# george-gca/sr-pytorch-lightning

Measured on AMD Instinct MI355X. Metric: SR training throughput, LR patches/s (48x48 LR x4, fwd+bwd+Adam), higher is better.
Workload: dtype bf16; 1 GPU; edsr_baseline x4, 48x48 LR patches, batch 256/GPU, train step (L1 + Adam); global_batch=256, parallelism=dp1, hip_graph=full

## Files before the change

sr-pytorch-lightning_amd/csrc/hr_tail.hip:

```cpp
#include "srk_common.h"

namespace {

SRK_DEV void sub_of(int a, int d, int& i, int& s) {
  const int ap = a + d;
  i = ap & 1;
  s = (ap - i) >> 1;
}

struct Wts {
  const float* wt; const float* bt; const float* wu; const float* bu;
  int O, C, Ci;
};

SRK_DEV float sum16(float v) {
  v += __shfl_xor(v, 8, 64);
  v += __shfl_xor(v, 4, 64);
  v += __shfl_xor(v, 2, 64);
  v += __shfl_xor(v, 1, 64);
  return v;
}

SRK_DEV float collapse_w(const Wts& p, int sub, int o, int a, int b, int ci, int dy0, int dy1, int dx0, int dx1, int fy, int fx) {
  float acc = 0.f;
  for (int dy = dy0; dy <= dy1; ++dy) {
    int i, sy; sub_of(a, dy, i, sy);
    const int ey = fy - sy;
    if (ey < -1 || ey > 1) continue;
    for (int dx = dx0; dx <= dx1; ++dx) {
      int j, sx; sub_of(b, dx, j, sx);
      const int ex = fx - sx;
      if (ex < -1 || ex > 1) continue;
      const float* wt = p.wt + (size_t)o * p.C * 9 + (dy + 1) * 3 + (dx + 1);
      const float* wu = p.wu + ((size_t)(i * 2 + j) * p.Ci + ci) * 9 + (ey + 1) * 3 + (ex + 1);
      for (int c0 = sub; c0 < p.C; c0 += 64) {
        float x[4], y[4];
#pragma unroll
        for (int k = 0; k < 4; ++k) {
          const int c = c0 + 16 * k;
          const bool ok = c < p.C;
          x[k] = ok ? wt[(size_t)c * 9] : 0.f;
          y[k] = ok ? wu[(size_t)c * 4 * p.Ci * 9] : 0.f;
        }
#pragma unroll
        for (int k = 0; k < 4; ++k)
          if (c0 + 16 * k < p.C) acc += x[k] * y[k];
      }
    }
  }
  return sum16(acc);
}
SRK_DEV float collapse_b(const Wts& p, int sub, int o, int a, int b, int dy0, int dy1, int dx0, int dx1) {
  float acc = 0.f;
  if (p.bu) {
    for (int dy = dy0; dy <= dy1; ++dy) {
      int i, sy; sub_of(a, dy, i, sy);
      for (int dx = dx0; dx <= dx1; ++dx) {
        int j, sx; sub_of(b, dx, j, sx);
        const float* wt = p.wt + (size_t)o * p.C * 9 + (dy + 1) * 3 + (dx + 1);
        for (int c = sub; c < p.C; c += 16) acc += wt[(size_t)c * 9] * p.bu[c * 4 + i * 2 + j];
      }
    }
  }
  return sum16(acc);
}

__global__ __launch_bounds__(256) void hrtail_collapse_kernel(const srk_hrtail_args a) {
  const Wts p{a.wt, a.bt, a.wu, a.bu, a.O, a.C, a.Ci};
  const int O = a.O, Ci = a.Ci;
  const int n_eff = 4 * O * Ci * 25, n_edge = 4 * 2 * O * Ci * 5, n_cor = 4 * O * Ci;
  const int n_b = 4 * O + 4 * 2 * O + 4 * O;
  const int sub = threadIdx.x & 15;
  int t = blockIdx.x * 16 + (threadIdx.x >> 4);
  if (t >= n_eff + n_edge + n_cor + n_b) t = n_eff + n_edge + n_cor + n_b;
  float v = 0.f;
  float* dst = nullptr;
  if (t < n_eff) {
    const int f = t % 25, ci = (t / 25) % Ci, k = t / (25 * Ci);
    v = collapse_w(p, sub, k >> 2, (k >> 1) & 1, k & 1, ci, -1, 1, -1, 1, f / 5 - 2, f % 5 - 2);
    dst = a.weff + t;
  } else if (t < n_eff + n_edge) {
    const int u = t - n_eff;
    const int tt = u % 5, ci = (u / 5) % Ci, kk = (u / (5 * Ci)) % (2 * O), ty = u / (5 * Ci * 2 * O);
    const int o = kk >> 1, q = kk & 1;
    if (ty == 0) v = collapse_w(p, sub, o, 0, q, ci, -1, -1, -1, 1, 0, tt - 2);
    else if (ty == 1) v = collapse_w(p, sub, o, 1, q, ci, 1, 1, -1, 1, 0, tt - 2);
    else if (ty == 2) v = collapse_w(p, sub, o, q, 0, ci, -1, 1, -1, -1, tt - 2, 0);
    else v = collapse_w(p, sub, o, q, 1, ci, -1, 1, 1, 1, tt - 2, 0);
    dst = a.wedge + u;
  } else if (t < n_eff + n_edge + n_cor) {
    const int u = t - n_eff - n_edge;
    const int ci = u % Ci, o = (u / Ci) % O, c = u / (Ci * O);
    const int ca = c >> 1, cb = c & 1;
    v = collapse_w(p, sub, o, ca, cb, ci, ca ? 1 : -1, ca ? 1 : -1, cb ? 1 : -1, cb ? 1 : -1, 0, 0);
    dst = a.wcor + u;
  } else if (t < n_eff + n_edge + n_cor + n_b) {
    const int w = t - n_eff - n_edge - n_cor;
    if (w < 4 * O) {
      const int k = w;
      v = (a.bt ? a.bt[k >> 2] : 0.f) + collapse_b(p, sub, k >> 2, (k >> 1) & 1, k & 1, -1, 1, -1, 1);
      dst = a.beff + k;
    } else if (w < 4 * O + 8 * O) {
      const int u = w - 4 * O, kk = u % (2 * O), ty = u / (2 * O), o = kk >> 1, q = kk & 1;
      if (ty == 0) v = collapse_b(p, sub, o, 0, q, -1, -1, -1, 1);
      else if (ty == 1) v = collapse_b(p, sub, o, 1, q, 1, 1, -1, 1);
      else if (ty == 2) v = collapse_b(p, sub, o, q, 0, -1, 1, -1, -1);
      else v = collapse_b(p, sub, o, q, 1, -1, 1, 1, 1);
      dst = a.bedge + u;
    } else {
      const int u = w - 12 * O, o = u % O, c = u / O, ca = c >> 1, cb = c & 1;
      v = collapse_b(p, sub, o, ca, cb, ca ? 1 : -1, ca ? 1 : -1, cb ? 1 : -1, cb ? 1 : -1);
      dst = a.bcor + u;
    }
  }
  if (dst && sub == 0) *dst = v;
}

template <int DT> SRK_DEV float ld_act(const void* base, size_t idx) {
  return DTraits<DT>::to_f32(reinterpret_cast<const typename DTraits<DT>::elem*>(base)[idx]);
}

constexpr int MAXO = 4;
SRK_DEV float wave_total(float v) {
#pragma unroll
  for (int m = 32; m >= 1; m >>= 1) v += __shfl_xor(v, m, 64);
  return v;
}
struct EdgeGeo {
  int ty, len; bool row;
  int fix_lr, fix_hr;
};
SRK_DEV EdgeGeo edge_geo(int ty, int H, int W) {
  EdgeGeo e;
  e.ty = ty; e.row = ty < 2; e.len = e.row ? W : H;
  e.fix_lr = ty == 0 ? 0 : ty == 1 ? H - 1 : ty == 2 ? 0 : W - 1;
  e.fix_hr = ty == 0 ? 0 : ty == 1 ? 2 * H - 1 : ty == 2 ? 0 : 2 * W - 1;
  return e;
}
SRK_DEV void stage_copy256(float* __restrict__ dst, const float* __restrict__ src, int n) {
  int i = threadIdx.x;
  for (; i + 256 * 7 < n; i += 256 * 8) {
    float v[8];
#pragma unroll
    for (int k = 0; k < 8; ++k) v[k] = src[i + 256 * k];
#pragma unroll
    for (int k = 0; k < 8; ++k) dst[i + 256 * k] = v[k];
  }
  float v[8];
#pragma unroll
  for (int k = 0; k < 8; ++k) v[k] = i + 256 * k < n ? src[i + 256 * k] : 0.f;
#pragma unroll
  for (int k = 0; k < 8; ++k)
    if (i + 256 * k < n) dst[i + 256 * k] = v[k];
}
template <int DT>
SRK_DEV void stage_line(const srk_hrtail_args& a, const EdgeGeo& e, int n, float* Xl, int pitch) {
  typedef DTraits<DT> Tr;
  const int Ci = a.Ci;
  if ((Ci & 7) == 0 && (a.x_pitch & 7) == 0) {
    const int nch = Ci >> 3, total = (e.len + 4) * nch;
    for (int i0 = threadIdx.x; i0 < total; i0 += 256 * 4) {
      i32x4 raw[4];
#pragma unroll
      for (int u = 0; u < 4; ++u) {
        const int i = i0 + 256 * u;
        const int sp = i / nch, c8 = i - sp * nch, s = sp - 2;
        raw[u] = i32x4{0, 0, 0, 0};
        if (i < total && s >= 0 && s < e.len) {
          const int yy = e.row ? e.fix_lr : s, xx = e.row ? s : e.fix_lr;
          raw[u] = gload16(reinterpret_cast<const typename Tr::elem*>(a.x) + ((size_t)(n * a.H + yy) * a.W + xx) * a.x_pitch + c8 * 8);
        }
      }
#pragma unroll
      for (int u = 0; u < 4; ++u) {
        const int i = i0 + 256 * u;
        if (i >= total) continue;
        const int sp = i / nch, c8 = i - sp * nch;
        const int w4[4] = {raw[u].x, raw[u].y, raw[u].z, raw[u].w};
        float v[8];
#pragma unroll
        for (int k = 0; k < 4; ++k) unpack2<DT>((uint32_t)w4[k], v[2 * k], v[2 * k + 1]);
#pragma unroll
        for (int k = 0; k < 8; ++k) Xl[sp * pitch + c8 * 8 + k] = v[k];
      }
    }
    return;
  }
  for (int i = threadIdx.x; i < (e.len + 4) * Ci; i += 256) {
    const int s = i / Ci - 2, ci = i % Ci;
    float v = 0.f;
    if (s >= 0 && s < e.len) {
      const int yy = e.row ? e.fix_lr : s, xx = e.row ? s : e.fix_lr;
      v = ld_act<DT>(a.x, ((size_t)(n * a.H + yy) * a.W + xx) * a.x_pitch + ci);
    }
    Xl[(s + 2) * pitch + ci] = v;
  }
}

template <int DT>
__global__ __launch_bounds__(256) void hrtail_edge_fwd_kernel(const srk_hrtail_args a, int phase) {
  const int H = a.H, W = a.W, O = a.O, Ci = a.Ci, H2 = 2 * H, W2 = 2 * W;
  const int n = blockIdx.x;
  const EdgeGeo e = edge_geo(2 * phase + blockIdx.y, H, W);
  extern __shared__ __attribute__((aligned(16))) char smem_raw[];
  const int pitch = Ci + 1;
  float* const Xl = reinterpret_cast<float*>(smem_raw);
  float* const Wl = Xl + (size_t)(e.len + 4) * pitch;
  stage_line<DT>(a, e, n, Xl, pitch);
  stage_copy256(Wl, a.wedge + (size_t)e.ty * 2 * O * Ci * 5, 2 * O * Ci * 5);
  __syncthreads();
  const size_t oplane = (size_t)H2 * W2;
  float* const out = a.out + (size_t)n * O * oplane;
  for (int idx = threadIdx.x + 256 * blockIdx.z; idx < 2 * e.len * O; idx += 256 * gridDim.z) {
    const int p = idx % (2 * e.len), o = idx / (2 * e.len);
    const int s = p >> 1, q = p & 1;
    const float* const w = Wl + (size_t)(o * 2 + q) * Ci * 5;
    const float* const x = Xl + (size_t)s * pitch;
    float a0 = a.bedge[e.ty * 2 * O + o * 2 + q], a1 = 0.f, a2 = 0.f, a3 = 0.f, a4 = 0.f;
    for (int ci = 0; ci < Ci; ++ci) {
      a0 += w[ci * 5 + 0] * x[0 * pitch + ci]; a1 += w[ci * 5 + 1] * x[1 * pitch + ci]; a2 += w[ci * 5 + 2] * x[2 * pitch + ci];
      a3 += w[ci * 5 + 3] * x[3 * pitch + ci]; a4 += w[ci * 5 + 4] * x[4 * pitch + ci];
    }
    float acc = ((a0 + a1) + (a2 + a3)) + a4;
    if (!e.row && (p == 0 || p == 2 * e.len - 1)) {
      const int ca = p == 0 ? 0 : 1, cb = e.ty == 2 ? 0 : 1, c = ca * 2 + cb;
      float cc = a.bcor[c * O + o];
      const float* const xc = Xl + (size_t)(s + 2) * pitch;
      for (int ci = 0; ci < Ci; ++ci) cc += a.wcor[((size_t)c * O + o) * Ci + ci] * xc[ci];
      acc -= cc;
    }
    const size_t at = e.row ? (size_t)e.fix_hr * W2 + p : (size_t)p * W2 + e.fix_hr;
    out[(size_t)o * oplane + at] -= acc;
  }
}

template <int DT>
__global__ __launch_bounds__(256) void hrtail_edge_bwd_x_kernel(const srk_hrtail_args a, int phase) {
  typedef DTraits<DT> Tr;
  const int H = a.H, W = a.W, O = a.O, Ci = a.Ci, H2 = 2 * H, W2 = 2 * W;
  const int n = blockIdx.x;
  const bool shared_line = phase == 0 ? H == 1 : W == 1;
  if (shared_line && blockIdx.y == 1) return;
  extern __shared__ __attribute__((aligned(16))) char smem_raw[];
  const size_t gplane = (size_t)H2 * W2;
  const float* const g = a.g + (size_t)n * O * gplane;
  for (int rep = 0; rep < (shared_line ? 2 : 1); ++rep) {
  const EdgeGeo e = edge_geo(2 * phase + (shared_line ? rep : (int)blockIdx.y), H, W);
  float* const Gl = reinterpret_cast<float*>(smem_raw);
  float* const Wl = Gl + (size_t)2 * O * (e.len + 4);
  __syncthreads();
  for (int i0 = threadIdx.x; i0 < 2 * O * (e.len + 4); i0 += 256 * 4) {
    float v[4];
#pragma unroll
    for (int u = 0; u < 4; ++u) {
      const int i = i0 + 256 * u;
      const int kk = i / (e.len + 4), s = i % (e.len + 4) - 2, o = kk >> 1, q = kk & 1;
      v[u] = 0.f;
      if (i < 2 * O * (e.len + 4) && s >= 0 && s < e.len)
        v[u] = e.row ? g[(size_t)o * gplane + (size_t)e.fix_hr * W2 + 2 * s + q] : g[(size_t)o * gplane + (size_t)(2 * s + q) * W2 + e.fix_hr];
    }
#pragma unroll
    for (int u = 0; u < 4; ++u)
      if (i0 + 256 * u < 2 * O * (e.len + 4)) Gl[i0 + 256 * u] = v[u];
  }
  stage_copy256(Wl, a.wedge + (size_t)e.ty * 2 * O * Ci * 5, 2 * O * Ci * 5);
  __syncthreads();
  const int nch = (Ci + 7) >> 3;
  const bool vec = (Ci & 7) == 0 && (a.dx_pitch & 7) == 0;
  for (int idx = threadIdx.x + 256 * blockIdx.z; idx < e.len * nch; idx += 256 * gridDim.z) {
    const int c8 = idx % nch, s = idx / nch;
    float corr[8];
#pragma unroll
    for (int k = 0; k < 8; ++k) corr[k] = 0.f;
    for (int kk = 0; kk < 2 * O; ++kk) {
      const float* const gl = Gl + (size_t)kk * (e.len + 4) + s + 2;
      float gv[5];
#pragma unroll
      for (int tt = 0; tt < 5; ++tt) gv[tt] = gl[2 - tt];
#pragma unroll
      for (int k = 0; k < 8; ++k) {
        const int ci = c8 * 8 + k;
        if (ci < Ci) {
          const float* const w = Wl + ((size_t)kk * Ci + ci) * 5;
#pragma unroll
          for (int tt = 0; tt < 5; ++tt) corr[k] += w[tt] * gv[tt];
        }
      }
    }
    if (!e.row && (s == 0 || s == e.len - 1)) {
      for (int ca = 0; ca < 2; ++ca) {
        if (!(ca ? s == e.len - 1 : s == 0)) continue;
        const int cb = e.ty == 2 ? 0 : 1, c = ca * 2 + cb;
        const size_t at = (size_t)(ca ? H2 - 1 : 0) * W2 + e.fix_hr;
        for (int o = 0; o < O; ++o) {
          const float gc = g[(size_t)o * gplane + at];
#pragma unroll
          for (int k = 0; k < 8; ++k)
            if (c8 * 8 + k < Ci) corr[k] -= a.wcor[((size_t)c * O + o) * Ci + c8 * 8 + k] * gc;
        }
      }
    }
    const int yy = e.row ? e.fix_lr : s, xx = e.row ? s : e.fix_lr;
    typename Tr::elem* const d = reinterpret_cast<typename Tr::elem*>(a.dx) + ((size_t)(n * H + yy) * W + xx) * a.dx_pitch + c8 * 8;
    if (vec) {
      const i32x4 raw = *reinterpret_cast<const i32x4*>(d);
      const int w4[4] = {raw.x, raw.y, raw.z, raw.w};
      int o4[4];
#pragma unroll
      for (int k = 0; k < 4; ++k) {
        float f0, f1;
        unpack2<DT>((uint32_t)w4[k], f0, f1);
        o4[k] = (int)pack2<DT>(f0 - corr[2 * k], f1 - corr[2 * k + 1]);
      }
      *reinterpret_cast<i32x4*>(d) = i32x4{o4[0], o4[1], o4[2], o4[3]};
    } else {
#pragma unroll
      for (int k = 0; k < 8; ++k)
        if (c8 * 8 + k < Ci) d[k] = Tr::from_f32(Tr::to_f32(d[k]) - corr[k]);
    }
  }
  }
}

constexpr int EW_MAXLEN = 512;
template <int DT>
__global__ __launch_bounds__(256) void hrtail_edge_bwd_w_kernel(const srk_hrtail_args a, int nchunks, int ew_chunk) {
  const int H = a.H, W = a.W, O = a.O, Ci = a.Ci, H2 = 2 * H, W2 = 2 * W;
  const int ty = blockIdx.y, chunk = blockIdx.x;
  const int n0 = chunk * ew_chunk, n1 = min(a.N, n0 + ew_chunk);
  const int ncombo = ty < 4 ? 2 * O * 5 : O;
  const size_t gplane = (size_t)H2 * W2;
  float* const dst = a.scratch + ((size_t)ty * nchunks + chunk) * (size_t)(2 * MAXO * 5) * (Ci + 1);
  extern __shared__ __attribute__((aligned(16))) char smem_raw[];
  float* const Xl = reinterpret_cast<float*>(smem_raw);
  if (ty >= 4) {
    if (blockIdx.z != 0) return;
    const int c = ty - 4, ca = c >> 1, cbb = c & 1;
    const int Py = ca ? H2 - 1 : 0, Px = cbb ? W2 - 1 : 0, yy = ca ? H - 1 : 0, xx = cbb ? W - 1 : 0;
    for (int item = threadIdx.x; item < ncombo * (Ci + 1); item += 256) {
      const int ci = item % (Ci + 1), o = item / (Ci + 1);
      float acc = 0.f;
      for (int n = n0; n < n1; ++n) {
        const float gv = a.g[((size_t)n * O + o) * gplane + (size_t)Py * W2 + Px];
        const float xv = ci < Ci ? ld_act<DT>(a.x, ((size_t)(n * H + yy) * W + xx) * a.x_pitch + ci) : 1.f;
        acc += gv * xv;
      }
      dst[item] = acc;
    }
    return;
  }
  const bool rowedge = ty < 2;
  const int len = rowedge ? W : H;
  float* const Gl = Xl + (size_t)(len + 4) * Ci;
  constexpr int MAXIT = (2 * MAXO * 5 * 65 + 255) / 256;
  const int nitems = ncombo * (Ci + 1);
  const int ipb = (nitems + gridDim.z - 1) / gridDim.z, item0 = blockIdx.z * ipb, item1 = min(nitems, item0 + ipb);
  float acc[MAXIT];
#pragma unroll
  for (int k = 0; k < MAXIT; ++k) acc[k] = 0.f;
  for (int n = n0; n < n1; ++n) {
    __syncthreads();
    stage_line<DT>(a, edge_geo(ty, H, W), n, Xl, Ci);
    for (int i = threadIdx.x; i < 2 * O * len; i += 256) {
      const int kk = i / len, s = i % len, o = kk >> 1, q = kk & 1;
      const float* const g = a.g + ((size_t)n * O + o) * gplane;
      Gl[i] = rowedge ? g[(size_t)(ty == 0 ? 0 : H2 - 1) * W2 + 2 * s + q] : g[(size_t)(2 * s + q) * W2 + (ty == 2 ? 0 : W2 - 1)];
    }
    __syncthreads();
#pragma unroll
    for (int k = 0; k < MAXIT; ++k) {
      const int item = item0 + threadIdx.x + k * 256;
      if (item >= item1) break;
      const int ci = item % (Ci + 1), cb = item / (Ci + 1), tt = cb % 5, kk = cb / 5;
      const float* const gr = Gl + kk * len;
      float t0 = 0.f, t1 = 0.f, t2 = 0.f, t3 = 0.f;
      int p = 0;
      if (ci < Ci) {
        const float* const xr = Xl + (size_t)tt * Ci + ci;
        for (; p + 3 < len; p += 4) {
          t0 += gr[p] * xr[(size_t)p * Ci]; t1 += gr[p + 1] * xr[(size_t)(p + 1) * Ci];
          t2 += gr[p + 2] * xr[(size_t)(p + 2) * Ci]; t3 += gr[p + 3] * xr[(size_t)(p + 3) * Ci];
        }
        for (; p < len; ++p) t0 += gr[p] * xr[(size_t)p * Ci];
      } else if (tt == 2) {
        for (; p + 3 < len; p += 4) { t0 += gr[p]; t1 += gr[p + 1]; t2 += gr[p + 2]; t3 += gr[p + 3]; }
        for (; p < len; ++p) t0 += gr[p];
      }
      acc[k] += (t0 + t1) + (t2 + t3);
    }
  }
#pragma unroll
  for (int k = 0; k < MAXIT; ++k) {
    const int item = item0 + threadIdx.x + k * 256;
    if (item < item1) dst[item] = acc[k];
  }
}

__global__ __launch_bounds__(256) void hrtail_edge_reduce_kernel(const srk_hrtail_args a, int nchunks) {
  const int O = a.O, Ci = a.Ci;
  const int per = 2 * MAXO * 5 * (Ci + 1);
  const int t = blockIdx.x * 256 + threadIdx.x;
  const int n_edge = 4 * 2 * O * 5 * (Ci + 1), n_cor = 4 * O * (Ci + 1);
  if (t >= n_edge + n_cor) return;
  int ty, item;
  if (t < n_edge) { ty = t / (2 * O * 5 * (Ci + 1)); item = t % (2 * O * 5 * (Ci + 1)); }
  else { const int u = t - n_edge; ty = 4 + u / (O * (Ci + 1)); item = u % (O * (Ci + 1)); }
  const float* const src = a.scratch + (size_t)ty * nchunks * per + item;
  float s0 = 0.f, s1 = 0.f, s2 = 0.f, s3 = 0.f;
  int c = 0;
  for (; c + 3 < nchunks; c += 4) {
    s0 += src[(size_t)c * per]; s1 += src[(size_t)(c + 1) * per]; s2 += src[(size_t)(c + 2) * per]; s3 += src[(size_t)(c + 3) * per];
  }
  for (; c < nchunks; ++c) s0 += src[(size_t)c * per];
  const float s = (s0 + s1) + (s2 + s3);
  const int ci = item % (Ci + 1), cb = item / (Ci + 1);
  if (ty < 4) {
    const int tt = cb % 5, kk = cb / 5;
    if (ci < Ci) a.eedge[(((size_t)ty * 2 * O + kk) * Ci + ci) * 5 + tt] = s;
    else if (tt == 2) a.e0[ty * 2 * O + kk] = s;
  } else {
    if (ci < Ci) a.ecor[((size_t)(ty - 4) * O + cb) * Ci + ci] = s;
    else a.k0[(ty - 4) * O + cb] = s;
  }
}

struct Gr {
  const float* r; const float* r0; const float* ee; const float* e0; const float* ec; const float* k0;
  int O, Ci;
};
SRK_DEV int row_type(int a, int dy) { return (a == 0 && dy == -1) ? 0 : ((a == 1 && dy == 1) ? 1 : -1); }
SRK_DEV int col_type(int b, int dx) { return (b == 0 && dx == -1) ? 2 : ((b == 1 && dx == 1) ? 3 : -1); }
SRK_DEV float g_w(const Gr& q, int o, int a, int b, int dy, int dx, int ci, int fy, int fx) {
  float v = q.r[(((size_t)(o * 4 + a * 2 + b)) * q.Ci + ci) * 25 + (fy + 2) * 5 + (fx + 2)];
  const int rt = row_type(a, dy), ct = col_type(b, dx);
  if (rt >= 0 && fy == 0) v -= q.ee[(((size_t)rt * 2 * q.O + o * 2 + b) * q.Ci + ci) * 5 + fx + 2];
  if (ct >= 0 && fx == 0) v -= q.ee[(((size_t)ct * 2 * q.O + o * 2 + a) * q.Ci + ci) * 5 + fy + 2];
  if (rt >= 0 && ct >= 0 && fy == 0 && fx == 0) v += q.ec[((size_t)(a * 2 + b) * q.O + o) * q.Ci + ci];
  return v;
}
SRK_DEV float g_b(const Gr& q, int o, int a, int b, int dy, int dx) {
  float v = q.r0[o * 4 + a * 2 + b];
  const int rt = row_type(a, dy), ct = col_type(b, dx);
  if (rt >= 0) v -= q.e0[rt * 2 * q.O + o * 2 + b];
  if (ct >= 0) v -= q.e0[ct * 2 * q.O + o * 2 + a];
  if (rt >= 0 && ct >= 0) v += q.k0[(a * 2 + b) * q.O + o];
  return v;
}

__global__ __launch_bounds__(256) void hrtail_expand_kernel(const srk_hrtail_args a) {
  const Gr q{a.r, a.r0, a.eedge, a.e0, a.ecor, a.k0, a.O, a.Ci};
  const int O = a.O, C = a.C, Ci = a.Ci;
  const int n_wu = 4 * C * Ci * 9, n_bu = 4 * C, n_bt = O;
  const int nb_thread = (n_wu + n_bu + n_bt + 255) / 256;
  if ((int)blockIdx.x >= nb_thread) {
    const int t = ((int)blockIdx.x - nb_thread) * 4 + (threadIdx.x >> 6), lane = threadIdx.x & 63;
    if (t >= O * C * 9) return;
    const int d = t % 9, c = (t / 9) % C, o = t / (9 * C);
    const int dy = d / 3 - 1, dx = d % 3 - 1;
    float acc = 0.f;
    for (int pa = 0; pa < 2; ++pa) {
      int i, sy; sub_of(pa, dy, i, sy);
      for (int pb = 0; pb < 2; ++pb) {
        int j, sx; sub_of(pb, dx, j, sx);
        const int cu = c * 4 + i * 2 + j;
        if (a.bu && lane == 0) acc += g_b(q, o, pa, pb, dy, dx) * a.bu[cu];
        for (int ci = lane; ci < Ci; ci += 64)
#pragma unroll
          for (int e = 0; e < 9; ++e)
            acc += g_w(q, o, pa, pb, dy, dx, ci, sy + e / 3 - 1, sx + e % 3 - 1) * a.wu[((size_t)cu * Ci + ci) * 9 + e];
      }
    }
    acc = wave_total(acc);
    if (lane == 0) a.dwt[t] = acc;
    return;
  }
  int t = blockIdx.x * 256 + threadIdx.x;
  if (t < n_wu) {
    const int e = t % 9, ci = (t / 9) % Ci, cu = t / (9 * Ci), c = cu >> 2, i = (cu >> 1) & 1, j = cu & 1;
    const int ey = e / 3 - 1, ex = e % 3 - 1;
    float acc = 0.f;
    for (int pa = 0; pa < 2; ++pa)
      for (int dy = -1; dy <= 1; ++dy) {
        int ii, sy; sub_of(pa, dy, ii, sy);
        if (ii != i) continue;
        for (int pb = 0; pb < 2; ++pb)
          for (int dx = -1; dx <= 1; ++dx) {
            int jj, sx; sub_of(pb, dx, jj, sx);
            if (jj != j) continue;
            for (int o = 0; o < O; ++o)
              acc += a.wt[((size_t)o * C + c) * 9 + (dy + 1) * 3 + dx + 1] * g_w(q, o, pa, pb, dy, dx, ci, sy + ey, sx + ex);
          }
      }
    a.dwu[t] = acc;
    return;
  }
  t -= n_wu;
  if (t < n_bu) {
    if (!a.dbu) return;
    const int cu = t, c = cu >> 2, i = (cu >> 1) & 1, j = cu & 1;
    float acc = 0.f;
    for (int pa = 0; pa < 2; ++pa)
      for (int dy = -1; dy <= 1; ++dy) {
        int ii, sy; sub_of(pa, dy, ii, sy);
        if (ii != i) continue;
        for (int pb = 0; pb < 2; ++pb)
          for (int dx = -1; dx <= 1; ++dx) {
            int jj, sx; sub_of(pb, dx, jj, sx);
            if (jj != j) continue;
            for (int o = 0; o < O; ++o) acc += a.wt[((size_t)o * C + c) * 9 + (dy + 1) * 3 + dx + 1] * g_b(q, o, pa, pb, dy, dx);
          }
      }
    a.dbu[cu] = acc;
    return;
  }
  t -= n_bu;
  if (t < n_bt && a.dbt) a.dbt[t] = a.r0[t * 4] + a.r0[t * 4 + 1] + a.r0[t * 4 + 2] + a.r0[t * 4 + 3];
}

int check_common(const srk_hrtail_args* a, const char* who) {
  SRK_CHECK_ARG(a, "%s: null argument", who);
  SRK_CHECK_ARG(a->O >= 1 && a->O <= MAXO && a->C >= 1 && a->Ci >= 1, "%s: O=%d (1..%d) C=%d Ci=%d", who, a->O, MAXO, a->C, a->Ci);
  return 0;
}
int check_act(const srk_hrtail_args* a, const char* who) {
  SRK_CHECK_ARG(a->N > 0 && a->H > 0 && a->W > 0, "%s: bad dims N=%d H=%d W=%d", who, a->N, a->H, a->W);
  SRK_CHECK_ARG(a->dtype == SRK_BF16 || a->dtype == SRK_F16, "%s: 16-bit activations only", who);
  SRK_CHECK_ARG((long long)a->N * a->O * 4 * a->H * a->W < (1ll << 31), "%s: output too large", who);
  return 0;
}

}

extern "C" int srk_hrtail_collapse(const srk_hrtail_args* a, srk_stream_t stream) {
  if (int rc = check_common(a, "srk_hrtail_collapse")) return rc;
  SRK_CHECK_ARG(a->wt && a->wu && a->weff && a->beff && a->wedge && a->bedge && a->wcor && a->bcor, "srk_hrtail_collapse: null pointer");
  const int total = 4 * a->O * a->Ci * 25 + 4 * 2 * a->O * a->Ci * 5 + 4 * a->O * a->Ci + 16 * a->O;
  hipLaunchKernelGGL(hrtail_collapse_kernel, dim3((unsigned)((total + 15) / 16)), dim3(256), 0, reinterpret_cast<hipStream_t>(stream), *a);
  SRK_LAUNCH_CHECK();
  return 0;
}

static unsigned edge_split(int N) {
  const int z = (512 + 2 * N - 1) / (2 * N);
  return (unsigned)(z < 1 ? 1 : (z > 8 ? 8 : z));
}

template <typename K> static int edge_lds_attr(K kernel, const char* who) {
  const hipError_t e = hipFuncSetAttribute(reinterpret_cast<const void*>(kernel), hipFuncAttributeMaxDynamicSharedMemorySize, 160 * 1024);
  if (e != hipSuccess) { srk_set_error("%s: cannot reserve LDS: %s", who, hipGetErrorString(e)); return (int)e; }
  return 0;
}

extern "C" int srk_hrtail_edge_fwd(const srk_hrtail_args* a, srk_stream_t stream) {
  if (int rc = check_common(a, "srk_hrtail_edge_fwd")) return rc;
  if (int rc = check_act(a, "srk_hrtail_edge_fwd")) return rc;
  SRK_CHECK_ARG(a->x && a->out && a->wedge && a->bedge && a->wcor && a->bcor, "srk_hrtail_edge_fwd: null pointer");
  const int len = a->H > a->W ? a->H : a->W;
  const size_t lds = ((size_t)(len + 4) * (a->Ci + 1) + (size_t)2 * a->O * a->Ci * 5) * 4;
  SRK_CHECK_ARG(lds <= 160 * 1024, "srk_hrtail_edge_fwd: edge of %d pixels x %d channels does not fit the LDS", len, a->Ci);
  static const int rc0 = edge_lds_attr(&hrtail_edge_fwd_kernel<SRK_BF16>, "srk_hrtail_edge_fwd");
  static const int rc1 = edge_lds_attr(&hrtail_edge_fwd_kernel<SRK_F16>, "srk_hrtail_edge_fwd");
  if (rc0 || rc1) return rc0 ? rc0 : rc1;
  hipStream_t st = reinterpret_cast<hipStream_t>(stream);
  for (int phase = 0; phase < 2; ++phase) {
    if (a->dtype == SRK_BF16) hipLaunchKernelGGL(hrtail_edge_fwd_kernel<SRK_BF16>, dim3((unsigned)a->N, 2, edge_split(a->N)), dim3(256), lds, st, *a, phase);
    else hipLaunchKernelGGL(hrtail_edge_fwd_kernel<SRK_F16>, dim3((unsigned)a->N, 2, edge_split(a->N)), dim3(256), lds, st, *a, phase);
    SRK_LAUNCH_CHECK();
  }
  return 0;
}

extern "C" int srk_hrtail_edge_bwd_x(const srk_hrtail_args* a, srk_stream_t stream) {
  if (int rc = check_common(a, "srk_hrtail_edge_bwd_x")) return rc;
  if (int rc = check_act(a, "srk_hrtail_edge_bwd_x")) return rc;
  SRK_CHECK_ARG(a->g && a->dx && a->wedge && a->wcor, "srk_hrtail_edge_bwd_x: null pointer");
  const int len = a->H > a->W ? a->H : a->W;
  const size_t lds = ((size_t)2 * a->O * (len + 4) + (size_t)2 * a->O * a->Ci * 5) * 4;
  SRK_CHECK_ARG(lds <= 160 * 1024, "srk_hrtail_edge_bwd_x: edge of %d pixels does not fit the LDS", len);
  static const int rc0 = edge_lds_attr(&hrtail_edge_bwd_x_kernel<SRK_BF16>, "srk_hrtail_edge_bwd_x");
  static const int rc1 = edge_lds_attr(&hrtail_edge_bwd_x_kernel<SRK_F16>, "srk_hrtail_edge_bwd_x");
  if (rc0 || rc1) return rc0 ? rc0 : rc1;
  hipStream_t st = reinterpret_cast<hipStream_t>(stream);
  for (int phase = 0; phase < 2; ++phase) {
    if (a->dtype == SRK_BF16) hipLaunchKernelGGL(hrtail_edge_bwd_x_kernel<SRK_BF16>, dim3((unsigned)a->N, 2, edge_split(a->N)), dim3(256), lds, st, *a, phase);
    else hipLaunchKernelGGL(hrtail_edge_bwd_x_kernel<SRK_F16>, dim3((unsigned)a->N, 2, edge_split(a->N)), dim3(256), lds, st, *a, phase);
    SRK_LAUNCH_CHECK();
  }
  return 0;
}

static int ew_chunk_of(int N) { return N <= 64 ? 1 : (N + 63) / 64; }

extern "C" long long srk_hrtail_scratch_floats(int N, int Ci) {
  const int ewc = ew_chunk_of(N);
  const long long nchunks = (N + ewc - 1) / ewc;
  return 8 * nchunks * (long long)(2 * MAXO * 5) * (Ci + 1);
}

extern "C" int srk_hrtail_edge_bwd_w(const srk_hrtail_args* a, srk_stream_t stream) {
  if (int rc = check_common(a, "srk_hrtail_edge_bwd_w")) return rc;
  if (int rc = check_act(a, "srk_hrtail_edge_bwd_w")) return rc;
  SRK_CHECK_ARG(a->x && a->g && a->scratch && a->eedge && a->e0 && a->ecor && a->k0, "srk_hrtail_edge_bwd_w: null pointer");
  const int ewc = ew_chunk_of(a->N);
  const int nchunks = (a->N + ewc - 1) / ewc;
  const unsigned nz = nchunks * 8 >= 512 ? 2 : (nchunks * 8 >= 256 ? 4 : 8);
  const int len = a->H > a->W ? a->H : a->W;
  SRK_CHECK_ARG(a->Ci <= 64 && len <= EW_MAXLEN, "srk_hrtail_edge_bwd_w: Ci=%d (<= 64) edge length %d (<= %d)", a->Ci, len, EW_MAXLEN);
  const size_t lds = ((size_t)(len + 4) * a->Ci + (size_t)2 * a->O * len) * 4;
  hipStream_t st = reinterpret_cast<hipStream_t>(stream);
  static const hipError_t attr0 = hipFuncSetAttribute(reinterpret_cast<const void*>(&hrtail_edge_bwd_w_kernel<SRK_BF16>), hipFuncAttributeMaxDynamicSharedMemorySize, 160 * 1024);
  static const hipError_t attr1 = hipFuncSetAttribute(reinterpret_cast<const void*>(&hrtail_edge_bwd_w_kernel<SRK_F16>), hipFuncAttributeMaxDynamicSharedMemorySize, 160 * 1024);
  if (attr0 != hipSuccess || attr1 != hipSuccess) { srk_set_error("srk_hrtail_edge_bwd_w: cannot reserve LDS"); return (int)(attr0 != hipSuccess ? attr0 : attr1); }
  if (a->dtype == SRK_BF16) hipLaunchKernelGGL(hrtail_edge_bwd_w_kernel<SRK_BF16>, dim3((unsigned)nchunks, 8, nz), dim3(256), lds, st, *a, nchunks, ewc);
  else hipLaunchKernelGGL(hrtail_edge_bwd_w_kernel<SRK_F16>, dim3((unsigned)nchunks, 8, nz), dim3(256), lds, st, *a, nchunks, ewc);
  SRK_LAUNCH_CHECK();
  const int total = (4 * 2 * a->O * 5 + 4 * a->O) * (a->Ci + 1);
  hipLaunchKernelGGL(hrtail_edge_reduce_kernel, dim3((unsigned)((total + 255) / 256)), dim3(256), 0, st, *a, nchunks);
  SRK_LAUNCH_CHECK();
  return 0;
}

extern "C" int srk_hrtail_expand(const srk_hrtail_args* a, srk_stream_t stream) {
  if (int rc = check_common(a, "srk_hrtail_expand")) return rc;
  SRK_CHECK_ARG(a->wt && a->wu && a->r && a->r0 && a->eedge && a->e0 && a->ecor && a->k0 && a->dwt && a->dwu, "srk_hrtail_expand: null pointer");
  const int per_thread = 4 * a->C * a->Ci * 9 + 4 * a->C + a->O, per_wave = a->O * a->C * 9;
  const int nblocks = (per_thread + 255) / 256 + (per_wave + 3) / 4;
  hipLaunchKernelGGL(hrtail_expand_kernel, dim3((unsigned)nblocks), dim3(256), 0, reinterpret_cast<hipStream_t>(stream), *a);
  SRK_LAUNCH_CHECK();
  return 0;
}
```

Before: 49920 LR patches/s.

## Specialize HR-tail edge kernels on output count and restage weights in LDS

Adds a forward edge kernel templated on the output-channel count O. Each thread computes all O outputs for one pixel, using an interleaved LDS weight layout read with 16-byte LDS loads and packed f32x2 FMAs, and it stages the corner weights into LDS. The backward-x edge kernel now prefetches its dx load and its gradient, weight and corner data before the staging writes, loads weights with vector loads, and reads corner weights and gradients from LDS instead of global memory. The aim is to cut redundant LDS and global traffic and load latency in these small edge-correction kernels. The O-templated forward kernel only runs when the z split is 1, which holds for batch 256. The split kernel is kept for small batches, at the cost of more LDS and more code paths.

```diff
diff --git a/sr-pytorch-lightning_amd/csrc/hr_tail.hip b/sr-pytorch-lightning_amd/csrc/hr_tail.hip
--- a/sr-pytorch-lightning_amd/csrc/hr_tail.hip
+++ b/sr-pytorch-lightning_amd/csrc/hr_tail.hip
@@ -137,22 +137,6 @@
   e.fix_hr = ty == 0 ? 0 : ty == 1 ? 2 * H - 1 : ty == 2 ? 0 : 2 * W - 1;
   return e;
 }
-SRK_DEV void stage_copy256(float* __restrict__ dst, const float* __restrict__ src, int n) {
-  int i = threadIdx.x;
-  for (; i + 256 * 7 < n; i += 256 * 8) {
-    float v[8];
-#pragma unroll
-    for (int k = 0; k < 8; ++k) v[k] = src[i + 256 * k];
-#pragma unroll
-    for (int k = 0; k < 8; ++k) dst[i + 256 * k] = v[k];
-  }
-  float v[8];
-#pragma unroll
-  for (int k = 0; k < 8; ++k) v[k] = i + 256 * k < n ? src[i + 256 * k] : 0.f;
-#pragma unroll
-  for (int k = 0; k < 8; ++k)
-    if (i + 256 * k < n) dst[i + 256 * k] = v[k];
-}
 template <int DT>
 SRK_DEV void stage_line(const srk_hrtail_args& a, const EdgeGeo& e, int n, float* Xl, int pitch) {
   typedef DTraits<DT> Tr;
@@ -197,8 +181,120 @@
   }
 }
 
+typedef float __attribute__((ext_vector_type(2))) f32x2;
+
+SRK_DEV float ld_cor(const srk_hrtail_args& a, int cb, int i) {
+  const int per = a.O * a.Ci, ca = i / per;
+  return a.wcor[(size_t)(ca * 2 + cb) * per + (i - ca * per)];
+}
+
+template <int DT, int O>
+__global__ __launch_bounds__(256) void hrtail_edge_fwd_kernel(const srk_hrtail_args a, int phase) {
+  const int H = a.H, W = a.W, Ci = a.Ci, H2 = 2 * H, W2 = 2 * W;
+  const int n = blockIdx.x, tid = threadIdx.x;
+  const EdgeGeo e = edge_geo(2 * phase + blockIdx.y, H, W);
+  extern __shared__ __attribute__((aligned(16))) char smem_raw[];
+  constexpr int WP = (5 * O + 3) & ~3;
+  const int pitch = Ci + 1;
+  float* const Xl = reinterpret_cast<float*>(smem_raw);
+  float* const Wl = Xl + (((e.len + 4) * pitch + 3) & ~3);
+  float* const Cl = Wl + 2 * Ci * WP;
+  const int nw = 2 * O * Ci * 5, ncor = e.row ? 0 : 2 * O * Ci, cb = e.ty == 2 ? 0 : 1;
+  const float* const wsrc = a.wedge + (size_t)e.ty * nw;
+  auto w_at = [&](int i) {
+    const int tt = i % 5, r = i / 5, ci = r % Ci, kk = r / Ci;
+    return ((kk & 1) * Ci + ci) * WP + (tt < 4 ? (kk >> 1) * 4 + tt : 4 * O + (kk >> 1));
+  };
+  float wv[8], cw[2];
+#pragma unroll
+  for (int k = 0; k < 8; ++k) wv[k] = tid + 256 * k < nw ? wsrc[tid + 256 * k] : 0.f;
+#pragma unroll
+  for (int k = 0; k < 2; ++k) cw[k] = tid + 256 * k < ncor ? ld_cor(a, cb, tid + 256 * k) : 0.f;
+  stage_line<DT>(a, e, n, Xl, pitch);
+#pragma unroll
+  for (int k = 0; k < 8; ++k)
+    if (tid + 256 * k < nw) Wl[w_at(tid + 256 * k)] = wv[k];
+#pragma unroll
+  for (int k = 0; k < 2; ++k)
+    if (tid + 256 * k < ncor) Cl[tid + 256 * k] = cw[k];
+  for (int i = tid + 2048; i < nw; i += 256) Wl[w_at(i)] = wsrc[i];
+  for (int i = tid + 512; i < ncor; i += 256) Cl[i] = ld_cor(a, cb, i);
+  __syncthreads();
+  const size_t oplane = (size_t)H2 * W2;
+  float* const out = a.out + (size_t)n * O * oplane;
+  const int wave = __builtin_amdgcn_readfirstlane(tid >> 6), lane = tid & 63;
+  const int q = wave & 1;
+  const float* const wq = Wl + (size_t)q * Ci * WP;
+  float b0[O];
+#pragma unroll
+  for (int o = 0; o < O; ++o) b0[o] = a.bedge[e.ty * 2 * O + o * 2 + q];
+  for (int s = (wave >> 1) * 64 + lane; s < e.len; s += 128) {
+    const int p = 2 * s + q;
+    const size_t at = e.row ? (size_t)e.fix_hr * W2 + p : (size_t)p * W2 + e.fix_hr;
+    float old[O];
+#pragma unroll
+    for (int o = 0; o < O; ++o) old[o] = out[(size_t)o * oplane + at];
+    const float* const x = Xl + (size_t)s * pitch;
+    f32x2 a01[O], a23[O];
+    float a4[O];
+#pragma unroll
+    for (int o = 0; o < O; ++o) { a01[o] = f32x2{b0[o], 0.f}; a23[o] = f32x2{0.f, 0.f}; a4[o] = 0.f; }
+#pragma unroll 4
+    for (int ci = 0; ci < Ci; ++ci) {
+      float w[WP];
+#pragma unroll
+      for (int v = 0; v < WP / 4; ++v) {
+        const i32x4 t = lds_read16(reinterpret_cast<const char*>(wq + ci * WP + 4 * v));
+        w[4 * v] = __int_as_float(t.x); w[4 * v + 1] = __int_as_float(t.y); w[4 * v + 2] = __int_as_float(t.z); w[4 * v + 3] = __int_as_float(t.w);
+      }
+      const f32x2 x01 = f32x2{x[ci], x[pitch + ci]}, x23 = f32x2{x[2 * pitch + ci], x[3 * pitch + ci]};
+      const float x4 = x[4 * pitch + ci];
+#pragma unroll
+      for (int o = 0; o < O; ++o) {
+        a01[o] += f32x2{w[4 * o], w[4 * o + 1]} * x01;
+        a23[o] += f32x2{w[4 * o + 2], w[4 * o + 3]} * x23;
+        a4[o] += w[4 * O + o] * x4;
+      }
+    }
+    float res[O];
+#pragma unroll
+    for (int o = 0; o < O; ++o) res[o] = ((a01[o].x + a01[o].y) + (a23[o].x + a23[o].y)) + a4[o];
+    if (!e.row && (p == 0 || p == 2 * e.len - 1)) {
+      const int ca = p == 0 ? 0 : 1, c = ca * 2 + cb;
+      const float* const xc = x + 2 * pitch;
+      const float* const cl = Cl + (size_t)ca * O * Ci;
+      float cc[O];
+#pragma unroll
+      for (int o = 0; o < O; ++o) cc[o] = a.bcor[c * O + o];
+      for (int ci = 0; ci < Ci; ++ci)
+#pragma unroll
+        for (int o = 0; o < O; ++o) cc[o] += cl[o * Ci + ci] * xc[ci];
+#pragma unroll
+      for (int o = 0; o < O; ++o) res[o] -= cc[o];
+    }
+#pragma unroll
+    for (int o = 0; o < O; ++o) out[(size_t)o * oplane + at] = old[o] - res[o];
+  }
+}
+
+SRK_DEV void stage_copy256(float* __restrict__ dst, const float* __restrict__ src, int n) {
+  int i = threadIdx.x;
+  for (; i + 256 * 7 < n; i += 256 * 8) {
+    float v[8];
+#pragma unroll
+    for (int k = 0; k < 8; ++k) v[k] = src[i + 256 * k];
+#pragma unroll
+    for (int k = 0; k < 8; ++k) dst[i + 256 * k] = v[k];
+  }
+  float v[8];
+#pragma unroll
+  for (int k = 0; k < 8; ++k) v[k] = i + 256 * k < n ? src[i + 256 * k] : 0.f;
+#pragma unroll
+  for (int k = 0; k < 8; ++k)
+    if (i + 256 * k < n) dst[i + 256 * k] = v[k];
+}
 template <int DT>
-__global__ __launch_bounds__(256) void hrtail_edge_fwd_kernel(const srk_hrtail_args a, int phase) {
+__global__ __launch_bounds__(256) void hrtail_edge_fwd_split_kernel(const srk_hrtail_args a, int phase) {
   const int H = a.H, W = a.W, O = a.O, Ci = a.Ci, H2 = 2 * H, W2 = 2 * W;
   const int n = blockIdx.x;
   const EdgeGeo e = edge_geo(2 * phase + blockIdx.y, H, W);
@@ -238,37 +334,76 @@
 __global__ __launch_bounds__(256) void hrtail_edge_bwd_x_kernel(const srk_hrtail_args a, int phase) {
   typedef DTraits<DT> Tr;
   const int H = a.H, W = a.W, O = a.O, Ci = a.Ci, H2 = 2 * H, W2 = 2 * W;
-  const int n = blockIdx.x;
+  const int n = blockIdx.x, tid = threadIdx.x;
+  constexpr int nt = 256;
   const bool shared_line = phase == 0 ? H == 1 : W == 1;
   if (shared_line && blockIdx.y == 1) return;
   extern __shared__ __attribute__((aligned(16))) char smem_raw[];
   const size_t gplane = (size_t)H2 * W2;
   const float* const g = a.g + (size_t)n * O * gplane;
+  const int nch = (Ci + 7) >> 3;
+  const bool vec = (Ci & 7) == 0 && (a.dx_pitch & 7) == 0;
   for (int rep = 0; rep < (shared_line ? 2 : 1); ++rep) {
   const EdgeGeo e = edge_geo(2 * phase + (shared_line ? rep : (int)blockIdx.y), H, W);
+  const int ng = 2 * O * (e.len + 4), nw = 2 * O * Ci * 5, ncor = e.row ? 0 : 2 * O * Ci, cb = e.ty == 2 ? 0 : 1;
   float* const Gl = reinterpret_cast<float*>(smem_raw);
-  float* const Wl = Gl + (size_t)2 * O * (e.len + 4);
+  float* const Wl = Gl + ((ng + 3) & ~3);
+  float* const Cl = Wl + nw;
+  float* const Gc = Cl + 2 * O * Ci;
+  const float* const wsrc = a.wedge + (size_t)e.ty * nw;
+  const bool w16 = (nw & 3) == 0 && (reinterpret_cast<uintptr_t>(wsrc) & 15) == 0;
+  const int total = e.len * nch, stride = nt * (int)gridDim.z;
+  int idx = tid + nt * (int)blockIdx.z;
+  auto dx_of = [&](int item) {
+    const int c8 = item % nch, s = item / nch;
+    const int yy = e.row ? e.fix_lr : s, xx = e.row ? s : e.fix_lr;
+    return reinterpret_cast<typename Tr::elem*>(a.dx) + ((size_t)(n * H + yy) * W + xx) * a.dx_pitch + c8 * 8;
+  };
+  auto g_of = [&](int i) {
+    const int kk = i / (e.len + 4), s = i % (e.len + 4) - 2, o = kk >> 1, q = kk & 1;
+    if (i >= ng || s < 0 || s >= e.len) return 0.f;
+    return e.row ? g[(size_t)o * gplane + (size_t)e.fix_hr * W2 + 2 * s + q] : g[(size_t)o * gplane + (size_t)(2 * s + q) * W2 + e.fix_hr];
+  };
+  auto gc_of = [&](int i) {
+    return g[(size_t)(i % O) * gplane + (size_t)(i / O ? H2 - 1 : 0) * W2 + e.fix_hr];
+  };
   __syncthreads();
-  for (int i0 = threadIdx.x; i0 < 2 * O * (e.len + 4); i0 += 256 * 4) {
-    float v[4];
-#pragma unroll
-    for (int u = 0; u < 4; ++u) {
-      const int i = i0 + 256 * u;
-      const int kk = i / (e.len + 4), s = i % (e.len + 4) - 2, o = kk >> 1, q = kk & 1;
-      v[u] = 0.f;
-      if (i < 2 * O * (e.len + 4) && s >= 0 && s < e.len)
-        v[u] = e.row ? g[(size_t)o * gplane + (size_t)e.fix_hr * W2 + 2 * s + q] : g[(size_t)o * gplane + (size_t)(2 * s + q) * W2 + e.fix_hr];
-    }
-#pragma unroll
-    for (int u = 0; u < 4; ++u)
-      if (i0 + 256 * u < 2 * O * (e.len + 4)) Gl[i0 + 256 * u] = v[u];
-  }
-  stage_copy256(Wl, a.wedge + (size_t)e.ty * 2 * O * Ci * 5, 2 * O * Ci * 5);
+  i32x4 raw = i32x4{0, 0, 0, 0};
+  if (vec && idx < total) raw = gload16(dx_of(idx));
+  float gv4[4], cw[2], gcv = 0.f;
+  i32x4 wq[2];
+#pragma unroll
+  for (int u = 0; u < 4; ++u) gv4[u] = g_of(tid + nt * u);
+#pragma unroll
+  for (int u = 0; u < 2; ++u) {
+    const int i = (tid + nt * u) * 4;
+    wq[u] = w16 && i < nw ? gload16(wsrc + i) : i32x4{0, 0, 0, 0};
+    cw[u] = tid + nt * u < ncor ? ld_cor(a, cb, tid + nt * u) : 0.f;
+  }
+  if (!e.row && tid < 2 * O) gcv = gc_of(tid);
+#pragma unroll
+  for (int u = 0; u < 4; ++u)
+    if (tid + nt * u < ng) Gl[tid + nt * u] = gv4[u];
+#pragma unroll
+  for (int u = 0; u < 2; ++u) {
+    const int i = (tid + nt * u) * 4;
+    if (w16 && i < nw) *reinterpret_cast<i32x4*>(Wl + i) = wq[u];
+    if (tid + nt * u < ncor) Cl[tid + nt * u] = cw[u];
+  }
+  if (!e.row && tid < 2 * O) Gc[tid] = gcv;
+  for (int i = tid + nt * 4; i < ng; i += nt) Gl[i] = g_of(i);
+  if (w16) {
+    for (int i = (tid + nt * 2) * 4; i < nw; i += nt * 4) *reinterpret_cast<i32x4*>(Wl + i) = gload16(wsrc + i);
+  } else {
+    for (int i = tid; i < nw; i += nt) Wl[i] = wsrc[i];
+  }
+  for (int i = tid + nt * 2; i < ncor; i += nt) Cl[i] = ld_cor(a, cb, i);
+  for (int i = tid + nt; !e.row && i < 2 * O; i += nt) Gc[i] = gc_of(i);
   __syncthreads();
-  const int nch = (Ci + 7) >> 3;
-  const bool vec = (Ci & 7) == 0 && (a.dx_pitch & 7) == 0;
-  for (int idx = threadIdx.x + 256 * blockIdx.z; idx < e.len * nch; idx += 256 * gridDim.z) {
+  for (bool first = true; idx < total; idx += stride, first = false) {
     const int c8 = idx % nch, s = idx / nch;
+    typename Tr::elem* const d = dx_of(idx);
+    if (vec && !first) raw = gload16(d);
     float corr[8];
 #pragma unroll
     for (int k = 0; k < 8; ++k) corr[k] = 0.f;
@@ -277,33 +412,42 @@
       float gv[5];
 #pragma unroll
       for (int tt = 0; tt < 5; ++tt) gv[tt] = gl[2 - tt];
-#pragma unroll
-      for (int k = 0; k < 8; ++k) {
-        const int ci = c8 * 8 + k;
-        if (ci < Ci) {
-          const float* const w = Wl + ((size_t)kk * Ci + ci) * 5;
-#pragma unroll
-          for (int tt = 0; tt < 5; ++tt) corr[k] += w[tt] * gv[tt];
+      if ((Ci & 7) == 0) {
+        const float* const wp = Wl + ((size_t)kk * Ci + c8 * 8) * 5;
+        float w[40];
+#pragma unroll
+        for (int v = 0; v < 10; ++v) {
+          const i32x4 t = lds_read16(reinterpret_cast<const char*>(wp + 4 * v));
+          w[4 * v] = __int_as_float(t.x); w[4 * v + 1] = __int_as_float(t.y); w[4 * v + 2] = __int_as_float(t.z); w[4 * v + 3] = __int_as_float(t.w);
+        }
+#pragma unroll
+        for (int k = 0; k < 8; ++k)
+#pragma unroll
+          for (int tt = 0; tt < 5; ++tt) corr[k] += w[k * 5 + tt] * gv[tt];
+      } else {
+#pragma unroll
+        for (int k = 0; k < 8; ++k) {
+          const int ci = c8 * 8 + k;
+          if (ci < Ci) {
+            const float* const w = Wl + ((size_t)kk * Ci + ci) * 5;
+#pragma unroll
+            for (int tt = 0; tt < 5; ++tt) corr[k] += w[tt] * gv[tt];
+          }
         }
       }
     }
     if (!e.row && (s == 0 || s == e.len - 1)) {
       for (int ca = 0; ca < 2; ++ca) {
         if (!(ca ? s == e.len - 1 : s == 0)) continue;
-        const int cb = e.ty == 2 ? 0 : 1, c = ca * 2 + cb;
-        const size_t at = (size_t)(ca ? H2 - 1 : 0) * W2 + e.fix_hr;
         for (int o = 0; o < O; ++o) {
-          const float gc = g[(size_t)o * gplane + at];
+          const float gc = Gc[ca * O + o];
 #pragma unroll
           for (int k = 0; k < 8; ++k)
-            if (c8 * 8 + k < Ci) corr[k] -= a.wcor[((size_t)c * O + o) * Ci + c8 * 8 + k] * gc;
+            if (c8 * 8 + k < Ci) corr[k] -= Cl[((size_t)ca * O + o) * Ci + c8 * 8 + k] * gc;
         }
       }
     }
-    const int yy = e.row ? e.fix_lr : s, xx = e.row ? s : e.fix_lr;
-    typename Tr::elem* const d = reinterpret_cast<typename Tr::elem*>(a.dx) + ((size_t)(n * H + yy) * W + xx) * a.dx_pitch + c8 * 8;
     if (vec) {
-      const i32x4 raw = *reinterpret_cast<const i32x4*>(d);
       const int w4[4] = {raw.x, raw.y, raw.z, raw.w};
       int o4[4];
 #pragma unroll
@@ -551,20 +695,36 @@
   return 0;
 }
 
+typedef void (*edge_fwd_fn)(const srk_hrtail_args, int);
+template <int DT> static edge_fwd_fn edge_fwd_of(int O) {
+  return O == 1 ? hrtail_edge_fwd_kernel<DT, 1> : O == 2 ? hrtail_edge_fwd_kernel<DT, 2> : O == 3 ? hrtail_edge_fwd_kernel<DT, 3> : hrtail_edge_fwd_kernel<DT, 4>;
+}
+static int edge_fwd_lds_attrs() {
+  if (int rc = edge_lds_attr(&hrtail_edge_fwd_split_kernel<SRK_BF16>, "srk_hrtail_edge_fwd")) return rc;
+  if (int rc = edge_lds_attr(&hrtail_edge_fwd_split_kernel<SRK_F16>, "srk_hrtail_edge_fwd")) return rc;
+  for (int O = 1; O <= MAXO; ++O) {
+    if (int rc = edge_lds_attr(edge_fwd_of<SRK_BF16>(O), "srk_hrtail_edge_fwd")) return rc;
+    if (int rc = edge_lds_attr(edge_fwd_of<SRK_F16>(O), "srk_hrtail_edge_fwd")) return rc;
+  }
+  return 0;
+}
+
 extern "C" int srk_hrtail_edge_fwd(const srk_hrtail_args* a, srk_stream_t stream) {
   if (int rc = check_common(a, "srk_hrtail_edge_fwd")) return rc;
   if (int rc = check_act(a, "srk_hrtail_edge_fwd")) return rc;
   SRK_CHECK_ARG(a->x && a->out && a->wedge && a->bedge && a->wcor && a->bcor, "srk_hrtail_edge_fwd: null pointer");
   const int len = a->H > a->W ? a->H : a->W;
-  const size_t lds = ((size_t)(len + 4) * (a->Ci + 1) + (size_t)2 * a->O * a->Ci * 5) * 4;
-  SRK_CHECK_ARG(lds <= 160 * 1024, "srk_hrtail_edge_fwd: edge of %d pixels x %d channels does not fit the LDS", len, a->Ci);
-  static const int rc0 = edge_lds_attr(&hrtail_edge_fwd_kernel<SRK_BF16>, "srk_hrtail_edge_fwd");
-  static const int rc1 = edge_lds_attr(&hrtail_edge_fwd_kernel<SRK_F16>, "srk_hrtail_edge_fwd");
-  if (rc0 || rc1) return rc0 ? rc0 : rc1;
+  const size_t lds = ((((size_t)(len + 4) * (a->Ci + 1) + 3) & ~(size_t)3) + (size_t)2 * a->Ci * ((5 * a->O + 3) & ~3) + (size_t)2 * a->O * a->Ci) * 4;
+  const size_t lds_split = ((size_t)(len + 4) * (a->Ci + 1) + (size_t)2 * a->O * a->Ci * 5) * 4;
+  SRK_CHECK_ARG(lds <= 160 * 1024 && lds_split <= 160 * 1024, "srk_hrtail_edge_fwd: edge of %d pixels x %d channels does not fit the LDS", len, a->Ci);
+  static const int rc0 = edge_fwd_lds_attrs();
+  if (rc0) return rc0;
   hipStream_t st = reinterpret_cast<hipStream_t>(stream);
+  const unsigned z = edge_split(a->N);
+  const edge_fwd_fn kernel = z > 1 ? (a->dtype == SRK_BF16 ? hrtail_edge_fwd_split_kernel<SRK_BF16> : hrtail_edge_fwd_split_kernel<SRK_F16>)
+                                   : (a->dtype == SRK_BF16 ? edge_fwd_of<SRK_BF16>(a->O) : edge_fwd_of<SRK_F16>(a->O));
   for (int phase = 0; phase < 2; ++phase) {
-    if (a->dtype == SRK_BF16) hipLaunchKernelGGL(hrtail_edge_fwd_kernel<SRK_BF16>, dim3((unsigned)a->N, 2, edge_split(a->N)), dim3(256), lds, st, *a, phase);
-    else hipLaunchKernelGGL(hrtail_edge_fwd_kernel<SRK_F16>, dim3((unsigned)a->N, 2, edge_split(a->N)), dim3(256), lds, st, *a, phase);
+    hipLaunchKernelGGL(kernel, dim3((unsigned)a->N, 2, z), dim3(256), z > 1 ? lds_split : lds, st, *a, phase);
     SRK_LAUNCH_CHECK();
   }
   return 0;
@@ -575,15 +735,16 @@
   if (int rc = check_act(a, "srk_hrtail_edge_bwd_x")) return rc;
   SRK_CHECK_ARG(a->g && a->dx && a->wedge && a->wcor, "srk_hrtail_edge_bwd_x: null pointer");
   const int len = a->H > a->W ? a->H : a->W;
-  const size_t lds = ((size_t)2 * a->O * (len + 4) + (size_t)2 * a->O * a->Ci * 5) * 4;
+  const size_t lds = ((((size_t)2 * a->O * (len + 4) + 3) & ~(size_t)3) + (size_t)2 * a->O * a->Ci * 5 + (size_t)2 * a->O * a->Ci + 2 * a->O) * 4;
   SRK_CHECK_ARG(lds <= 160 * 1024, "srk_hrtail_edge_bwd_x: edge of %d pixels does not fit the LDS", len);
   static const int rc0 = edge_lds_attr(&hrtail_edge_bwd_x_kernel<SRK_BF16>, "srk_hrtail_edge_bwd_x");
   static const int rc1 = edge_lds_attr(&hrtail_edge_bwd_x_kernel<SRK_F16>, "srk_hrtail_edge_bwd_x");
   if (rc0 || rc1) return rc0 ? rc0 : rc1;
   hipStream_t st = reinterpret_cast<hipStream_t>(stream);
+  const unsigned z = edge_split(a->N);
   for (int phase = 0; phase < 2; ++phase) {
-    if (a->dtype == SRK_BF16) hipLaunchKernelGGL(hrtail_edge_bwd_x_kernel<SRK_BF16>, dim3((unsigned)a->N, 2, edge_split(a->N)), dim3(256), lds, st, *a, phase);
-    else hipLaunchKernelGGL(hrtail_edge_bwd_x_kernel<SRK_F16>, dim3((unsigned)a->N, 2, edge_split(a->N)), dim3(256), lds, st, *a, phase);
+    if (a->dtype == SRK_BF16) hipLaunchKernelGGL(hrtail_edge_bwd_x_kernel<SRK_BF16>, dim3((unsigned)a->N, 2, z), dim3(256), lds, st, *a, phase);
+    else hipLaunchKernelGGL(hrtail_edge_bwd_x_kernel<SRK_F16>, dim3((unsigned)a->N, 2, z), dim3(256), lds, st, *a, phase);
     SRK_LAUNCH_CHECK();
   }
   return 0;
```

New measurement: 50310 LR patches/s (median of 6 runs). About the same (+0.8%).
